# rst-tu-dortmund/mpc_local_planner

Hardware: AMD Instinct MI355X
Metric: MPC solves/sec (batched control cycles) at N=50 carlike (higher is better)
Workload: dtype f64

## Files before the change

mpc_local_planner_amd/csrc/mpc_capi.hip:

```cpp
#include <hip/hip_runtime.h>

#include <cstdio>
#include <cstdlib>
#include <cstring>
#include <new>
#include <string>
#include <vector>

#include "../../include/mpc_hip.h"
#include "mpc_core.hpp"
#include "mpc_problem.hpp"
#include "mpc_launch_plan.hpp"
#include "mpc_wave.hpp"
#include "mpc_solve_kernel.hpp"
#include "mpc_costmap.hpp"
#include "mpc_feasibility.hpp"
#include "mpc_grid_update.hpp"

namespace {

thread_local char g_err[512] = "";

void set_err(const char* what, hipError_t e) {
    snprintf(g_err, sizeof(g_err), "%s: %s", what, hipGetErrorString(e));
// ... 122 lines not shown
    c->model = MPC_MODEL_UNICYCLE;
    c->model_params[0] = 0.5;
    c->model_params[1] = 1.0;
    c->n = 20;
    c->dt_ref = 0.3;
    c->dt_free = 1;
    c->dt_lb = 0.0;
    c->dt_ub = 10.0;
    c->xf_fixed[0] = c->xf_fixed[1] = c->xf_fixed[2] = 1;
    c->collocation = MPC_COLLOC_FORWARD;
    c->objective = MPC_OBJ_MIN_TIME;
    c->u_lb[0] = -0.2; c->u_ub[0] = 0.4;
    c->u_lb[1] = -0.3; c->u_ub[1] = 0.3;
    for (int j = 0; j < 2; ++j) { c->du_lb[j] = -1e30; c->du_ub[j] = 1e30; }
    c->max_iter = 100;
    c->tol = 1e-8;
    c->mu_init = 0.1;
    c->precision = MPC_FP64;
    c->min_obstacle_dist = 0.5;
    c->force_inclusion_dist = 0.5;
    c->cutoff_dist = 2.0;
    c->footprint_kind = MPC_FOOTPRINT_POINT;
    c->max_obstacles = 0;
    c->max_vertices = 1;
    c->max_obstacle_rows = 4;
}

const char* mpc_last_error(void) { return g_err; }
int32_t mpc_version(void) { return 700; }

#ifdef MPC_PROFILE
int mpc_debug_profile(long long* out, int rows) {
#ifdef MPC_SPLIT_BUILD
    std::memset(out, 0, sizeof(long long) * 16 * (size_t)rows);
    hipError_t e = hipSuccess;
#define MPC_PROFILE_ADD(T, M) if (e == hipSuccess) e = mpc::solve_profile_add<T, M>(out, rows);
    MPC_PROFILE_ADD(double, 0) MPC_PROFILE_ADD(double, 1) MPC_PROFILE_ADD(double, 2) MPC_PROFILE_ADD(double, 3)
    MPC_PROFILE_ADD(float, 0) MPC_PROFILE_ADD(float, 1) MPC_PROFILE_ADD(float, 2) MPC_PROFILE_ADD(float, 3)
#undef MPC_PROFILE_ADD
    return (int)e;
#else
    return (int)hipMemcpyFromSymbol(out, HIP_SYMBOL(g_mpc_prof), sizeof(long long) * 16 * (size_t)rows, 0, hipMemcpyDeviceToHost);
#endif
}
#endif

int mpc_create(const mpc_config* cfg, int32_t max_batch, int32_t device, mpc_solver** out) {
    g_err[0] = 0;
    if (!cfg || !out || max_batch <= 0) { set_err("mpc_create: bad argument"); return MPC_EINVAL; }
    *out = nullptr;
    if (const char* why = mpc::config_error(*cfg)) { set_err(why); return MPC_EINVAL; }
    int ndev = 0;
    hipError_t e = hipGetDeviceCount(&ndev);
    if (e != hipSuccess || ndev <= 0) {
        set_err("mpc_create: no HIP device available (this library has no CPU fallback)");
        return MPC_ENODEV;
    }
    if (device < 0 || device >= ndev) { set_err("mpc_create: device index out of range"); return MPC_ENODEV; }
    HIP_TRY(hipSetDevice(device));
    const mpc::LaunchPlan plan = mpc::make_launch_plan(*cfg);
    if (const char* why = mpc::plan_error(plan)) { set_err(why); return MPC_EINVAL; }
    mpc_solver* s = new (std::nothrow) mpc_solver;
    if (!s) return MPC_ENOMEM;
    memset(s, 0, sizeof(*s));
    s->cfg = *cfg;
    s->plan = plan;
    mpc::fill_records(*cfg, s->P64, s->P32);
    s->device = device;
    s->max_batch = max_batch;
    const size_t n = cfg->n;
    hipError_t er = hipStreamCreateWithFlags(&s->stream, hipStreamNonBlocking);
    if (er == hipSuccess) er = hipEventCreate(&s->ev0);
    if (er == hipSuccess) er = hipEventCreate(&s->ev1);
    if (er == hipSuccess) er = hipEventCreate(&s->cev0);
    if (er == hipSuccess) er = hipEventCreate(&s->cev1);
// ... 605 lines not shown
```

mpc_local_planner_amd/csrc/mpc_solve_kernel.hpp:

```cpp
#pragma once
#include <hip/hip_runtime.h>
#include <cstddef>
#include <vector>

#include "../../include/mpc_hip.h"
#include "mpc_core.hpp"
#include "mpc_launch_plan.hpp"
#include "mpc_wave.hpp"

namespace mpc {

struct CandCtl {
    int n_cand;
    int* win;
    int* exited;
    int* it_sum;
    double* rec;
    int32_t* winner_out;
    int32_t* iters_total_out;
    int32_t* rows_dropped;
    double* dual;
    int dual_words;
    int dual_read;
};
// ... 192 lines not shown
    }
    return kern;
}

template <typename T, int MODEL>
hipError_t launch_solve(const SolveLaunch& a) {
    if (a.k.L.GSW > 0 && !a.gstage) return hipErrorInvalidConfiguration;
    auto kern = select_kernel<T, MODEL>(a.k);
    if (!kern) return hipErrorInvalidConfiguration;
    if (a.k.lds > 48u * 1024u) {
        hipError_t e = hipFuncSetAttribute(reinterpret_cast<const void*>(kern), hipFuncAttributeMaxDynamicSharedMemorySize, (int)a.k.lds);
        if (e != hipSuccess) return e;
    }
    hipLaunchKernelGGL(kern, dim3((unsigned)a.B * (unsigned)(a.cc.n_cand > 1 ? a.cc.n_cand : 1)), dim3(kWave), a.k.lds, a.stream, *static_cast<const Problem<T>*>(a.rec), a.k.L, a.B, a.x0, a.xf, a.u_prev, a.dt_prev,
                       a.x_init, a.u_init, a.dt_init, a.obst, a.n_grid, a.n_via, a.via, a.cc, a.iters_add, a.x_out, a.u_out, a.dt_out, a.status, a.iters, a.gstage, a.gslots, a.n_gslots,
                       static_cast<const Problem<T>*>(a.ptab), a.set_of);
    return hipSuccess;
}

template <typename T, int MODEL>
hipError_t solve_occupancy(const KernelChoice& k, int* out) {
    auto kern = select_kernel<T, MODEL>(k);
    if (!kern) return hipErrorInvalidConfiguration;
    if (k.lds > 48u * 1024u) {
        hipError_t e = hipFuncSetAttribute(reinterpret_cast<const void*>(kern), hipFuncAttributeMaxDynamicSharedMemorySize, (int)k.lds);
        if (e != hipSuccess) return e;
    }
    return hipOccupancyMaxActiveBlocksPerMultiprocessor(out, kern, kWave, k.lds);
}

#ifdef MPC_PROFILE
template <typename T, int MODEL>
hipError_t solve_profile_add(long long* acc, int rows) {
    std::vector<long long> b((size_t)16 * rows);
    hipError_t e = hipMemcpyFromSymbol(b.data(), HIP_SYMBOL(g_mpc_prof), sizeof(long long) * b.size(), 0, hipMemcpyDeviceToHost);
    for (size_t i = 0; e == hipSuccess && i < b.size(); ++i) acc[i] += b[i];
    return e;
}
#endif

#if defined(MPC_SPLIT_BUILD) && !defined(MPC_SOLVE_INST)
#ifdef MPC_PROFILE
#define MPC_EXTERN_PROFILE(T, M) extern template hipError_t solve_profile_add<T, M>(long long*, int);
#else
#define MPC_EXTERN_PROFILE(T, M)
#endif
#define MPC_EXTERN_LAUNCH(T, M) extern template hipError_t launch_solve<T, M>(const SolveLaunch&); extern template hipError_t solve_occupancy<T, M>(const KernelChoice&, int*); \
                                MPC_EXTERN_PROFILE(T, M)
MPC_EXTERN_LAUNCH(double, 0) MPC_EXTERN_LAUNCH(double, 1) MPC_EXTERN_LAUNCH(double, 2) MPC_EXTERN_LAUNCH(double, 3)
MPC_EXTERN_LAUNCH(float, 0) MPC_EXTERN_LAUNCH(float, 1) MPC_EXTERN_LAUNCH(float, 2) MPC_EXTERN_LAUNCH(float, 3)
#undef MPC_EXTERN_LAUNCH
#undef MPC_EXTERN_PROFILE
#endif

}
```

mpc_local_planner_amd/csrc/mpc_wave.hpp:

```cpp
#pragma once
#include <hip/hip_runtime.h>
#include <type_traits>

#include "mpc_core.hpp"
#include "mpc_dpp_blocks.inc"

#ifdef MPC_PROFILE
__device__ long long g_mpc_prof[4096][16];
#endif

#include "mpc_wave_layout.hpp"
#include "mpc_wave_debug.hpp"

namespace mpc {

template <typename T, int MODEL, int EXT = 1, bool OBST = true, int NSC = 0, bool GS = false, bool W2 = false>
struct IpmWave {
    static constexpr int NSTG = EXT ? NSTG_EXT : NSTG_BASE;
    static constexpr int NTRB = (MODEL == MODEL_KINEMATIC_BICYCLE || MODEL == MODEL_SIMPLE_CAR_FRONT) ? 4 : 3;
    static_assert(NSC == 0 || (EXT == 0 && !OBST), "the fixed layout exists for the headline instantiation only");
    static_assert(!GS || NSC == 0, "the fixed layout keeps its factorisation data in LDS");
    static_assert(!W2 || (!GS && EXT == 0 && !OBST), "the two-wave kernel exists for the headline instantiation in the LDS form only");
    using LayoutT = typename LayoutOf<NSC, NTRB, NSTG>::type;
    const Problem<T>& P;
    const LayoutT L;
    T* sm;
    T* gmb = nullptr;
    const int lane;
    T x0[3], xf[3], uprev[2], dtprev;
    T mu, rho, delta_last;
    T erho = T(0);
    bool row0_on, fail0;
    bool warm_guess = false;
    mutable int cnt_mult = -1, cnt_bmult = -1;
    mutable T inv_cnt_mult = T(1), inv_cnt_bmult = T(1);
    int nvia = 0;
    int flags;
#ifdef MPC_PROFILE
    mutable long long prof_mult = 0;
    mutable long long prof_loop = 0, prof_setup = 0, prof_fwd_loop = 0;
#endif
// ... 91 lines not shown
    }
    __device__ __forceinline__ T ut(int j, int k, T alpha) const {
        T u = F(L.U, j, k);
        if (alpha != T(0)) u += alpha * F(L.DU, j, k);
        return u;
    }

    __device__ __forceinline__ bool row_on(int r, int q) const { return ron(q) && (r > 0 || row0_on); }

    __device__ __forceinline__ T row_val(int UB, T d, int r, int q) const {
        const int n = L.n, j = q & 1;
        T ur = r < n - 1 ? F(UB, j, r) : T(0);
        const T up0 = uprev[0], up1 = uprev[1];
        T um = j ? up1 : up0;
        if (r > 0) um = F(UB, j, r - 1);
        T dtp = r > 0 ? d : dtprev;
        return slot_sign<T>(q) * ((ur - um) - P.rate_lim[q] * dtp);
    }
    __device__ __forceinline__ T row_jdz(int r, int q, T dd) const {
        const int n = L.n, j = q & 1;
        T dur = r < n - 1 ? F(L.DU, j, r) : T(0);
        T dum = r > 0 ? F(L.DU, j, r - 1) : T(0);
        return slot_sign<T>(q) * ((dur - dum) - (r > 0 ? P.rate_lim[q] * dd : T(0)));
    }

    __device__ __forceinline__ T push_interior(T v, T lb, T ub) const {
        T pl = t_min(Algo<T>::bound_push * t_max(T(1), t_abs(lb)), Algo<T>::bound_push * (ub - lb));
        T pu = t_min(Algo<T>::bound_push * t_max(T(1), t_abs(ub)), Algo<T>::bound_push * (ub - lb));
        return t_min(t_max(v, lb + pl), ub - pu);
    }

    __device__ __forceinline__ int local_lane() const { int l = lane; asm volatile("" : "+v"(l)); return l; }
#define MPC_PHASE_LANE const int lane = W2 ? this->local_lane() : this->lane; (void)lane;
    static constexpr bool kUniformScalars = W2;
    __device__ __forceinline__ static double uni_(double v) { return __hiloint2double(__builtin_amdgcn_readfirstlane(__double2hiint(v)), __builtin_amdgcn_readfirstlane(__double2loint(v))); }
    __device__ __forceinline__ static float uni_(float v) { return __int_as_float(__builtin_amdgcn_readfirstlane(__float_as_int(v))); }
    __device__ __attribute__((noinline)) static T pow_cold(T a, T b) { return t_pow(a, b); }
    __device__ __forceinline__ static T pow_(T a, T b) { if constexpr (W2) return pow_cold(a, b); else return t_pow(a, b); }
    __device__ __forceinline__ static void U(T& v) { if constexpr (kUniformScalars) v = uni_(v); }
    template <typename... Ts> __device__ __forceinline__ static void U(T& v, Ts&... rest) { U(v); U(rest...); }

#include "mpc_wave_rows.inc"
#include "mpc_wave_passes.inc"
#include "mpc_wave_sweeps.inc"
#include "mpc_wave_pit.inc"
#include "mpc_wave_step.inc"
#include "mpc_wave_solve.inc"
#undef MPC_PHASE_LANE
};

}
```

mpc_local_planner_amd/csrc/mpc_wave_debug.hpp:

```cpp
#pragma once

#ifdef MPC_ASM_MARK
#define MPC_MARK(name) asm volatile("; " name)
#else
#define MPC_MARK(name) do { } while (0)
#endif

#ifdef MPC_PROFILE
#define MPC_PROFILE_BEGIN \
        long long tk[8] = {0, 0, 0, 0, 0, 0, 0, 0}; int nfac = 0, ntrial = 0; \
        const long long t_begin = __builtin_readcyclecounter(); \
        const long long w_begin = wall_clock64();
#define MPC_TICK(i, stmt) { long long t0_ = __builtin_readcyclecounter(); stmt; tk[i] += __builtin_readcyclecounter() - t0_; }
#define MPC_PROFILE_COUNT(c) ++c
#define MPC_PROFILE_END \
        if (lane == 0 && blockIdx.x < 4096) { \
            long long* o = g_mpc_prof[blockIdx.x]; \
            o[0] = __builtin_readcyclecounter() - t_begin; o[1] = wall_clock64() - w_begin; o[2] = it; o[3] = nfac; o[4] = ntrial; \
            for (int i = 0; i < 8; ++i) o[5 + i] = tk[i]; \
            o[13] = prof_loop; o[14] = prof_setup; o[15] = prof_fwd_loop; if (prof_mult) o[10] = prof_mult;       \
        }
#else
#define MPC_PROFILE_BEGIN
#define MPC_TICK(i, stmt) { stmt; }
#define MPC_PROFILE_COUNT(c) do { } while (0)
#define MPC_PROFILE_END
#endif

#ifdef MPC_PIT_CHECK
#define MPC_DBG_PIT_CHECK \
                if (pit && (int)blockIdx.x < MPC_PIT_CHECK) { \
                    T dd1 = T(0), nu1[3] = {T(0), T(0), T(0)}, dd2 = T(0), nu2[3] = {T(0), T(0), T(0)}; \
                    const int g1c = backward_pit(delta, dc, dd1, nu1); sync(); \
                    const bool g1 = g1c > 0; \
                    if (g1) { forward_pit(dd1, nu1, delta); sync(); } \
                    T keepx = T(0), keepu = T(0), keepl = T(0); \
                    const int kk = lane < L.n - 1 ? lane : 0; \
                    keepx = F(L.DX, 2, kk); keepu = F(L.DU, 1, kk); keepl = F(L.LAMN, 2, kk); \
                    sync(); \
                    const bool g2 = backward_dpp(delta, dc, dd2, nu2); sync(); \
                    if (g2) { forward_states(dd2, nu2, delta); sync(); } \
                    const T ex = wave_max(t_abs(keepx - F(L.DX, 2, kk))), eu = wave_max(t_abs(keepu - F(L.DU, 1, kk))), el = wave_max(t_abs(keepl - F(L.LAMN, 2, kk))); \
                    const T sx = wave_max(t_abs(F(L.DX, 2, kk))), su = wave_max(t_abs(F(L.DU, 1, kk))), sl = wave_max(t_abs(F(L.LAMN, 2, kk))); \
                    if (lane == 0 && (g1 != g2 || ex > T(1e-7) * (sx + T(1e-3)) || eu > T(1e-7) * (su + T(1e-3)) || el > T(1e-7) * (sl + T(1e-3)))) \
                        printf("blk %d it %d try %d delta %.2e mu %.1e: pit ok %d (code %d) serial ok %d | dd %.9e vs %.9e | max diff dx %.2e (of %.2e) du %.2e (of %.2e) lam %.2e (of %.2e)\n", (int)blockIdx.x, it, ntry, (double)delta, (double)mu, \
                               (int)g1, g1c, (int)g2, (double)dd1, (double)dd2, (double)ex, (double)sx, (double)eu, (double)su, (double)el, (double)sl); \
                    sync(); \
                }
#else
#define MPC_DBG_PIT_CHECK
#endif

#ifdef MPC_NANCHECK
#define MPC_DBG_NANCHECK_FIELDS \
                if (blockIdx.x == MPC_NANCHECK && lane == 0) { \
                    const int offs[] = {L.X, L.U, L.LAM, L.LAMN, L.SR, L.YR, L.PL, L.PU, L.DX, L.DU, L.CC, L.TRIG, L.GAIN, L.STG, L.SC, L.VP, L.ZC, L.total}; \
                    const char* nm[] = {"X", "U", "LAM", "LAMN", "SR", "YR", "PL", "PU", "DX", "DU", "CC", "TRIG", "GAIN", "STG", "SC", "VP", "ZC"}; \
// ... 30 lines not shown
```

mpc_local_planner_amd/csrc/mpc_wave_passes.inc:

```

    __device__ __forceinline__ void eval_point(T d, T& theta_c, T& fobj, T alpha = T(0), bool trial = false) const {
        MPC_PHASE_LANE
        const int n = L.n;
        const T al = trial ? alpha : T(0);
        T th = T(0), fo = T(0);
        if (nM() > 0) {
            for_each_row([&](int k, int m) {
                if (oi(m, k) < 0) return;
                T og = T(0), oax = T(0), oay = T(0);
                if (trial) { og = OB_(0, m, k); oax = OB_(1, m, k); oay = OB_(2, m, k); }
                const T px = xt(0, k, al), py = xt(1, k, al), pth = fpline() ? xt(2, k, al) : T(0);
                T g, a3[3], hk, h3[3];
                obst_row3(k, m, px, py, pth, g, a3, hk, h3, d);
                T s = F(L.OS, m, k);
                if (erho > T(0)) {
                    const T ee = OE_(0, m, k), de = trial ? T(OE_(1, m, k)) : T(0);
                    if (trial) s += alpha * (-(og + s - ee) - obst_jdz(k, m, oax, oay) + de);
                    const T et = ee + (trial ? alpha * de : T(0));
                    th += t_abs(g + s - et);
                    fo += erho * et;
                    return;
                }
                if (trial) s += alpha * (-(og + s) - obst_jdz(k, m, oax, oay));
                th += t_abs(g + s);
// ... 57 lines not shown
            if (nM() > 0 && k >= 1 && k < n - 1) {
                for (int m0 = 0; m0 < nM(); m0 += kRowGroup) {
                RowCache oc;
                if (trial) ob_load<false>(m0, k, oc);
#pragma unroll
                for (int jm = 0; jm < kRowGroup; ++jm) {
                    const int m = m0 + jm;
                    if (m >= nM()) break;
                    if (oi(m, k) < 0) continue;
                    T s = F(L.OS, m, k);
                    if (erho > T(0)) {
                        const T ee = OE_(0, m, k), de = trial ? T(OE_(1, m, k)) : T(0);
                        if (trial) s += alpha * (-(oc.g[jm] + s - ee) - obst_jdz(k, m, oc.ax[jm], oc.ay[jm]) + de);
                        acc.mul(s); acc.mul(ee + (trial ? alpha * de : T(0)));
                        continue;
                    }
                    if (trial) s += alpha * (-(oc.g[jm] + s) - obst_jdz(k, m, oc.ax[jm], oc.ay[jm]));
                    acc.mul(s);
                }
                }
            }
        }
        if (lane == 0 && dtf()) { acc.mul(d - P.dt_lb); acc.mul(P.dt_ub - d); }
        if (lane == 0 && ball()) acc.mul(ball_slack(alpha, trial));
        return wave_sum(acc.value());
    }

    struct TrialRegs {
        T xk[3], dxk[3], xn[3], dxn[3], u[2], du[2], s[4], ds[4];
        T ulb[2], uub[2], dt_lb, dt_ub, nm1;
        bool stage, on[4], quad, mint, dtf;
        int k;
    };
    __device__ __forceinline__ bool trial_fast_ok() const { return EXT == 0 && !GS && !W2 && !OBST && !(sizeof(T) == 8 && NTRB > 3) && L.n <= kWave; }
    __device__ __forceinline__ void trial_setup(TrialRegs& r, T dd) const {
        MPC_PHASE_LANE
        const int n = L.n, k = lane;
        const T d = SCL(SC_D);
        r.k = k; r.stage = k < n - 1;
        r.quad = quad(); r.mint = mintime(); r.dtf = dtf(); r.nm1 = T(n - 1);
        r.dt_lb = P.dt_lb; r.dt_ub = P.dt_ub;
        for (int i = 0; i < 3; ++i) {
            r.xk[i] = r.dxk[i] = r.xn[i] = r.dxn[i] = T(0);
            if (r.stage) {
                r.xk[i] = F(L.X, i, k); r.xn[i] = F(L.X, i, k + 1);
                if (k > 0) r.dxk[i] = F(L.DX, i, k);
                if (k + 1 < n - 1 || !fx(i)) r.dxn[i] = F(L.DX, i, k + 1);
            }
        }
        for (int j = 0; j < 2; ++j) {
            r.ulb[j] = P.u_lb[j]; r.uub[j] = P.u_ub[j];
            r.u[j] = r.stage ? F(L.U, j, k) : T(0); r.du[j] = r.stage ? F(L.DU, j, k) : T(0);
        }
        for (int q = 0; q < 4; ++q) {
            r.on[q] = k < n && row_on(k, q);
            r.s[q] = T(1); r.ds[q] = T(0);
            if (r.on[q]) { const T s = F(L.SR, q, k); r.s[q] = s; r.ds[q] = -(row_val(L.U, d, k, q) + s) - row_jdz(k, q, dd); }
        }
    }
    __device__ __forceinline__ void trial_eval(const TrialRegs& r, T alpha, T d, T& th_out, T& fo_out, T& logs_out) const {
        MPC_PHASE_LANE
        T th = T(0), fo = T(0);
        LogAcc<T> acc;
        if (r.stage) {
            const T x0_ = r.xk[0] + alpha * r.dxk[0], x1_ = r.xk[1] + alpha * r.dxk[1];
            const T x2_ = r.k > 0 ? normalize_theta(r.xk[2] + alpha * r.dxk[2]) : r.xk[2];
            const T n0 = r.xn[0] + alpha * r.dxn[0], n1 = r.xn[1] + alpha * r.dxn[1];
            const T n2 = r.dxn[2] != T(0) ? normalize_theta(r.xn[2] + alpha * r.dxn[2]) : r.xn[2];
            const T v = r.u[0] + alpha * r.du[0], w = r.u[1] + alpha * r.du[1];
            T tr[4], tr2[2], f[3];
            model_trig_colloc<T, MODEL>(P, x2_, v, w, d, tr, tr2);
            colloc_f<T, MODEL>(P, tr, tr2, v, w, f);
            const T c0 = d * f[0] - (n0 - x0_), c1 = d * f[1] - (n1 - x1_), c2 = d * f[2] - normalize_theta(n2 - x2_);
            for (int i = 0; i < NTRB; ++i) F(L.TRIG, i, r.k) = tr[i];
            if (P.collocation == COLLOC_CN) { F(L.TRIG, NTRB, r.k) = tr2[0]; F(L.TRIG, NTRB + 1, r.k) = tr2[1]; }
            C_(0, r.k) = c0; C_(1, r.k) = c1; C_(2, r.k) = c2;
            th = t_abs(c0) + t_abs(c1) + t_abs(c2);
            if (r.quad) {
                const T xd0 = x0_ - xf[0], xd1 = x1_ - xf[1], xd2 = normalize_theta(x2_ - xf[2]);
                fo = (P.Q[0] * xd0 * xd0 + P.Q[1] * xd1 * xd1 + P.Q[2] * xd2 * xd2 + P.R[0] * v * v + P.R[1] * w * w) * (intf() ? d : T(1));
            }
            if (via()) { T vv, vg[3]; via_terms(r.k, x0_, x1_, x2_, vv, vg); fo += vv; }
// ... 347 lines not shown
```

mpc_local_planner_amd/csrc/mpc_wave_solve.inc:

```

    __device__ __forceinline__ T enter_restoration(T& dtheta) {
        const int n = L.n;
        erho = Algo<T>::elastic_rho;
        T esum = T(0), dth = T(0);
        for (int k = lane; k < n - 1; k += kWave) {
            if (k < 1) continue;
            for (int m = 0; m < nM(); ++m) {
                if (oi(m, k) < 0) continue;
                const T g = OB_(0, m, k);
                const T s_old = F(L.OS, m, k);
                const T s = t_max(t_max(-g, Algo<T>::clearance_slack_push), s_old);
                const T ee = t_max(g + s, mu / erho);
                const T y = t_max(t_min(F(L.OY, m, k), T(0.5) * erho), mu / s);
                F(L.OS, m, k) = s; F(L.OY, m, k) = y; OE_(0, m, k) = ee; OE_(1, m, k) = T(0);
                esum += ee;
                dth += t_abs(g + s - ee) - t_abs(g + s_old);
            }
        }
        esum = wave_sum(esum);
        dtheta = wave_sum(dth);
        sync();
        return erho * esum;
    }

    __device__ __forceinline__ SolveStats<T> solve() {
        SolveStats<T> out;
        flags = (P.xf_fixed[0] ? 1 : 0) | (P.xf_fixed[1] ? 2 : 0) | (P.xf_fixed[2] ? 4 : 0) | (P.dt_free ? 8 : 0) | (P.objective == OBJ_QUADRATIC ? 16 : 0) |
                (P.has_Qf ? 32 : 0) | (P.rate_on[0] ? 64 : 0) | (P.rate_on[1] ? 128 : 0) | (P.rate_on[2] ? 256 : 0) | (P.rate_on[3] ? 512 : 0) | (P.ball ? 1024 : 0) | (P.via ? 2048 : 0) | ((P.n_obst > 0 && (P.footprint_kind == 2 || P.footprint_kind == 3 || P.footprint_kind == 4)) ? 4096 : 0) | (P.integral_form ? 8192 : 0) | (P.dyn_obst ? 16384 : 0) | (P.hess_mode ? 32768 : 0) | ((P.objective != OBJ_QUADRATIC || P.hybrid) ? 65536 : 0) | (P.costx ? 131072 : 0);
        flags = __builtin_amdgcn_readfirstlane(flags);
        nfix = (int)fx(0) + (int)fx(1) + (int)fx(2);
        row0_on = dtprev != T(0);
        if (iter_cap <= 0) iter_cap = P.max_iter;
        if (lane < 8) sm[L.ZC + lane] = lane == 4 ? T(1) : T(0);
        if constexpr (GS) {
            if (lane < 8) gw((unsigned)(GlobalStage::ZC + lane)) = lane == 4 ? T(1) : T(0);
            for (int k = lane - GlobalStage::kGuard; k < 4 * GlobalStage::tiles(L.NS) - GlobalStage::kGuard; k += kWave) {
#pragma unroll
                for (int j = 0; j < 6; ++j) TL_(TE_Z + j, k) = j == 3 ? T(1) : T(0);
            }
        }
        if (lane < 12) sm[L.ZI + lane] = lane == 6 ? T(1) : T(0);
        const bool pit = pit_enabled();
        init_point();
        U(mu, rho, delta_last); U(x0[0], x0[1], x0[2]); U(xf[0], xf[1], xf[2]); U(uprev[0], uprev[1], dtprev);
        T theta_c, fobj;
        eval_point(SCL(SC_D), theta_c, fobj);
        U(theta_c, fobj);
        sync();
        int it = 0, status = ST_MAX_ITER, n_acc = 0;
        const long long t_start = P.max_ticks > 0 ? (long long)wall_clock64() : 0ll;
        const T acc_tol = P.acc_tol;
        const int acc_it = P.acc_iter;
        T e0 = T(0), logs_cur = T(0), dc_mu = T(-1), dc_val = T(0);
        T last_alpha = T(0), last_ad = T(0);
        int jam_streak = 0;
        T jam_theta0 = T(0);
        bool endgame = false;
        T mu_max = Algo<T>::mu_max_fact * mu; U(mu_max);
        bool have_logs = false;
        const bool filter = P.line_search == 1;
        T fstate = T(-1);
        int nfilt = 0, fpos = 0;
        static_assert(Algo<T>::flt_cap == 16, "the filter's pairs sit in DPP rows 0 and 1");
        MPC_PROFILE_BEGIN
        while (true) {
            Err er;
            MPC_MARK("KKT_BEGIN");
            MPC_TICK(0, er = kkt_pass());
            U(er.rd, er.rp, er.cmin, er.cmax); U(er.csum, er.sum_mult, er.sum_bmult, er.theta); U(inv_cnt_mult, inv_cnt_bmult);
            MPC_MARK("KKT_END");
            if constexpr (OBST) {
                if (nM() > 0 && erho == T(0) && jam_streak >= Algo<T>::elastic_trigger && er.theta >= Algo<T>::elastic_prog * jam_theta0) {
                    T dth_rows;
                    fobj += enter_restoration(dth_rows);
                    theta_c += dth_rows;
                    rho = T(0); have_logs = false; jam_streak = 0;
                    nfilt = 0; fpos = 0;
                    er = kkt_pass();
                    U(er.rd, er.rp, er.cmin, er.cmax); U(er.csum, er.sum_mult, er.sum_bmult, er.theta); U(theta_c, fobj, erho);
                }
            }
            e0 = err_value(er, T(0)); U(e0);
            if (!t_finite(e0) || !t_finite(er.theta) || !t_finite(er.sum_mult) || !t_finite(er.csum)) { status = ST_NUMERICAL; break; }
            if (e0 <= P.tol) { status = ST_CONVERGED; break; }
            n_acc = (acc_it > 0 && e0 <= acc_tol) ? n_acc + 1 : 0;
            if (acc_it > 0 && n_acc >= acc_it) { status = ST_CONVERGED; break; }
            if (it >= iter_cap) { status = ST_MAX_ITER; break; }
            if (P.max_ticks > 0 && (long long)wall_clock64() - t_start > P.max_ticks) { status = ST_TIME_LIMIT; break; }
            if (win_ptr) {
                const int w = __builtin_amdgcn_readfirstlane(__hip_atomic_load(win_ptr, __ATOMIC_RELAXED, __HIP_MEMORY_SCOPE_AGENT));
                if (w < my_cand) { status = ST_SUPERSEDED; break; }
            }
            if (P.mu_strategy == 1 || endgame) {
                for (int guard = 0; guard < 50; ++guard) {
                    T emu = err_value(er, mu);
                    if (emu <= Algo<T>::kappa_eps * mu && mu > P.tol / T(10)) {
                        mu = t_max(P.tol / T(10), t_min(Algo<T>::kappa_mu * mu, pow_(mu, Algo<T>::theta_mu)));
                        rho = T(0);
                    } else break;
                }
            } else if (it > 0) {
                const T avg = er.csum * inv_cnt_bmult;
                const T a_ = T(1) - t_min(last_alpha, last_ad);
                const T sig = t_min(t_max(a_ * a_ * a_, Algo<T>::sigma_min), T(1));
                T mu_new = t_min(t_max(sig * avg, P.tol / T(10)), mu_max);
                mu_new = t_max(mu_new, t_min(mu, Algo<T>::mu_err_floor * e0));
                if (mu_new <= P.tol) { mu_new = P.tol; endgame = true; }
                if (mu_new != mu) { mu = mu_new; rho = T(0); }
            }
            U(mu, rho);
            MPC_MARK("BARRIER_BEGIN");
            MPC_TICK(1, stage_barrier_terms(); sync());
            MPC_MARK("BARRIER_END");
            T tau = t_max(Algo<T>::tau_min, T(1) - mu);
            if (mu != dc_mu) { dc_mu = mu; dc_val = nfix > 0 ? Algo<T>::delta_c * pow_(mu, Algo<T>::kappa_c) : T(0); }
            U(tau, dc_mu, dc_val);
            const T dc = dc_val;
            T delta = (fail0 && delta_last > T(0)) ? t_max(Algo<T>::delta_min, Algo<T>::kappa_minus * delta_last) : T(0);
            U(delta);
            const bool started_zero = delta == T(0);
            bool ok = false;
            Fwd fw;
            T dd = T(0), nu[3] = {T(0), T(0), T(0)}, curv = T(0);
            for (int ntry = 0; ntry <= 40; ++ntry) {
                bool good, used_pit = false;
                MPC_DBG_PIT_CHECK
                if (pit && mu > pit_floor()) {
                    int gp_;
                    MPC_TICK(2, gp_ = backward_pit(delta, dc, dd, nu); sync());
                    good = used_pit = gp_ > 0;
                    if (gp_ == 0) { MPC_TICK(2, good = backward_dpp(delta, dc, dd, nu); sync()); }
                } else { MPC_TICK(2, good = backward_dpp(delta, dc, dd, nu); sync()); }
                MPC_PROFILE_COUNT(nfac);
                MPC_DBG_NANCHECK_FIELDS
                U(dd, nu[0], nu[1], nu[2]);
                if (good) {
                    if (used_pit) { MPC_TICK(3, forward_pit(dd, nu, delta); sync()); }
                    else { MPC_TICK(3, forward_states(dd, nu, delta); sync()); }
                    MPC_DBG_NANCHECK_STEP
                    MPC_MARK("POST_BEGIN");
                    MPC_TICK(4, fw = post_pass(dd, nu, tau));
                    U(fw.hdz, fw.clam, fw.dz2, fw.dphi); U(fw.a_p, fw.a_d, fw.dzmax, fw.nunu);
                    MPC_MARK("POST_END");
                    good = fw.finite;
                    if (good) {
                        curv = -fw.hdz + fw.clam - dc * fw.nunu; U(curv);
                        ok = true; break;
                    }
                }
                if (delta == T(0)) delta = (delta_last == T(0)) ? Algo<T>::delta_first : t_max(Algo<T>::delta_min, Algo<T>::kappa_minus * delta_last);
                else delta *= (delta_last == T(0)) ? Algo<T>::kappa_plus_first : Algo<T>::kappa_plus;
                U(delta);
                if (delta > Algo<T>::delta_max) break;
            }
            if (!ok) { status = ST_LINSOLVE; break; }
            if constexpr (OBST) {
                if (nM() > 0 && erho == T(0)) {
                    if (fw.a_p < Algo<T>::elastic_ap && er.rp > T(1e-3)) { if (jam_streak == 0) jam_theta0 = er.theta; ++jam_streak; }
                    else jam_streak = 0;
                }
            }
            if (delta > T(0)) delta_last = delta;
            U(delta_last);
            if (started_zero) fail0 = delta > T(0);
            const T theta = er.theta;
            if (!filter && theta > T(0)) {
                T sigma = curv > T(0) ? T(1) : T(0);
                T rho_trial = (fw.dphi + T(0.5) * sigma * curv) / ((T(1) - Algo<T>::rho_frac) * theta);
                if (rho < rho_trial) rho = rho_trial + T(1);
                U(rho);
            }
            T phi0;
            if (!have_logs) { MPC_TICK(5, logs_cur = barrier_logs(SCL(SC_D), T(0), false, dd)); have_logs = true; U(logs_cur); }
            const T rho_ls = filter ? T(0) : rho;
            phi0 = fobj - mu * logs_cur + rho_ls * theta;
            T Dm = fw.dphi - rho_ls * theta;
            T theta_rows = theta - theta_c;
            T alpha = fw.a_p;
            U(phi0, Dm, theta_rows, alpha);
            T a_min = T(0), p_ph = T(0), p_th = T(0), theta_max = T(0), theta_min = T(0);
            if (filter) {
                T theta0 = rd_lane(fstate, 32);
                if (theta0 < T(0)) { theta0 = theta; if (lane == 32) fstate = theta; }
                if (mu != rd_lane(fstate, 33)) { nfilt = 0; fpos = 0; if (lane == 33) fstate = mu; }
                theta_max = Algo<T>::flt_thmax * t_max(T(1), theta0); theta_min = Algo<T>::flt_thmin * t_max(T(1), theta0);
                a_min = Algo<T>::flt_gth;
                if (fw.dphi < T(0)) {
                    a_min = t_min(a_min, Algo<T>::flt_gph * theta / (-fw.dphi));
                    if (theta <= theta_min) {
                        p_ph = pow_cold(-fw.dphi, Algo<T>::flt_sph); p_th = pow_cold(theta, Algo<T>::flt_sth);
                        a_min = t_min(a_min, Algo<T>::flt_delta * p_th / p_ph);
                    }
                }
                a_min = a_min * Algo<T>::flt_gal * fw.a_p;
                theta_max = uni_(theta_max); theta_min = uni_(theta_min); a_min = uni_(a_min); p_ph = uni_(p_ph); p_th = uni_(p_th);
            }
            bool accepted = false, sw_arm = false;
            const bool fast_trials = trial_fast_ok();
            TrialRegs tregs;
            if (fast_trials) { MPC_TICK(5, trial_setup(tregs, dd)); }
            T th_t = T(0), f_t = T(0), lg_t = T(0);
            for (int ls = 0; ls < Algo<T>::max_ls; ++ls) {
                if (ls > 0) { alpha *= T(0.5); U(alpha); }
                const bool below = filter && ls > 0 && alpha < a_min;
                T phit, tht;
                T d_t = SCL(SC_D) + (dtf() ? alpha * SCL(SC_DD) : T(0)); U(d_t);
                MPC_MARK("TRIAL_BEGIN");
                if (fast_trials) {
                    MPC_TICK(6, trial_eval(tregs, alpha, d_t, th_t, f_t, lg_t);
                             tht = th_t + (T(1) - alpha) * theta_rows;
                             phit = f_t - mu * lg_t + rho_ls * tht; sync());
                } else {
                    MPC_TICK(6, eval_point(d_t, th_t, f_t, alpha, true);
                             tht = th_t + (T(1) - alpha) * theta_rows;
                             lg_t = barrier_logs(d_t, alpha, true, dd);
                             phit = f_t - mu * lg_t + rho_ls * tht; sync());
                }
                MPC_MARK("TRIAL_END");
                MPC_PROFILE_COUNT(ntrial);
                U(th_t, f_t, lg_t, phit);
                if (!filter) {
                    if (t_finite(phit) && phit - phi0 - Algo<T>::ls_eps * t_abs(phi0) <= Algo<T>::eta_armijo * alpha * Dm) { accepted = true; break; }
                } else {
                    if (below) break;
                    U(tht);
                    bool okf = t_finite(phit) && tht <= theta_max;
                    if (okf) {
                        const T f_ph = __shfl_xor(fstate, 16);
                        const bool dominated = lane < nfilt && !(tht <= (T(1) - Algo<T>::flt_gth) * fstate || phit <= f_ph - Algo<T>::flt_gph * fstate);
                        okf = __builtin_amdgcn_ballot_w64(dominated) == 0ull;
                    }
                    if (okf) {
                        const bool switching = fw.dphi < T(0) && alpha * p_ph > Algo<T>::flt_delta * p_th;
                        if (theta <= theta_min && switching) {
                            if (phit - phi0 - Algo<T>::ls_eps * t_abs(phi0) <= Algo<T>::flt_eta * alpha * fw.dphi) { accepted = true; sw_arm = true; }
                        } else if (tht <= (T(1) - Algo<T>::flt_gth) * theta || phit <= phi0 - Algo<T>::flt_gph * theta) accepted = true;
                    }
                    if (accepted) break;
                }
            }
            if (filter) {
                if (accepted && !sw_arm) {
                    if (lane == fpos) fstate = theta;
                    if (lane == Algo<T>::flt_cap + fpos) fstate = phi0;
                    fpos = (fpos + 1) & (Algo<T>::flt_cap - 1); nfilt = nfilt < Algo<T>::flt_cap ? nfilt + 1 : Algo<T>::flt_cap;
                }
                if (!accepted) {
                    nfilt = 0; fpos = 0;
                    accepted = t_finite(f_t) && t_finite(lg_t);
                }
            }
            MPC_DBG_NANCHECK_LS_FAILED
            if (acc_tol > T(0) && (!accepted || alpha < T(1e-6) * fw.a_p) && e0 <= acc_tol) { status = ST_CONVERGED; break; }
            if (!accepted && alpha * fw.dzmax < T(1e-14)) { status = ST_LINESEARCH; break; }
            MPC_DBG_NANCHECK_LS
            MPC_MARK("ACCEPT_BEGIN");
            MPC_TICK(7, accept(alpha, fw.a_d); sync());
            MPC_MARK("ACCEPT_END");
            theta_c = th_t; fobj = f_t; logs_cur = lg_t;
            last_alpha = alpha; last_ad = fw.a_d;
            U(theta_c, fobj, logs_cur); U(last_alpha, last_ad);
            ++it;
        }
        MPC_PROFILE_END
        out.status = status; out.iters = it; out.kkt_error = e0; out.objective = fobj;
        return out;
    }
```

mpc_local_planner_amd/csrc/mpc_wave_step.inc:

```

    struct Fwd { T hdz, clam, dz2, dphi, a_p, a_d, dzmax, nunu; bool finite; };

    __device__ __forceinline__ void ftb_ratio(T ival, T dval, T& r) const { r = t_max(r, -dval * ival); }
    __device__ __forceinline__ T ftb_alpha(T r, T tau) const { return r > tau ? tau / r : T(1); }

    __device__ __forceinline__ Fwd post_pass(T dd, const T nu[3], T tau) const {
        MPC_PHASE_LANE
        const int n = L.n;
        const T d = SCL(SC_D);
        T hdz = T(0), clam = T(0), dz2 = T(0), dphi = T(0), r_p = T(0), r_d = T(0), dzmax = T(0);
        if (lane == 0) {
            if (dtf()) {
                T dl = d - P.dt_lb, du = P.dt_ub - d;
                T pl = SCL(SC_PDL), pu = SCL(SC_PDU);
                const T idl = t_rcp(dl), idu = t_rcp(du);
                T gb = -mu * idl + mu * idu;
                hdz += gb * dd; dphi += gb * dd;
                ftb_ratio(idl, dd, r_p); ftb_ratio(idu, -dd, r_p);
                ftb_ratio(t_rcp(pl), mu * idl - pl - (pl * idl) * dd, r_d);
                ftb_ratio(t_rcp(pu), mu * idu - pu + (pu * idu) * dd, r_d);
                dz2 += dd * dd; dzmax = t_max(dzmax, t_abs(dd));
            }
            if (mintime()) { hdz += T(n - 1) * dd; dphi += T(n - 1) * dd; }
            if (ball()) {
                const T jdz = ball_jdz(), s = SCL(SC_TS), y = SCL(SC_TY), res = SCL(SC_TG) + s;
                const T is = t_rcp(s);
                const T sig = y * is, ybar = mu * is + sig * res;
                const T ds = -res - jdz, dy = ybar + sig * jdz - y;
                hdz += ybar * jdz;
                dphi -= (mu * is) * ds;
                ftb_ratio(is, ds, r_p);
                ftb_ratio(t_rcp(y), dy, r_d);
            }
        }
        for (int k = lane; k < n; k += kWave) {
            if (k < n - 1) {
                for (int j = 0; j < 2; ++j) {
                    T u = F(L.U, j, k), du_ = F(L.DU, j, k);
                    T dl = u - P.u_lb[j], du = P.u_ub[j] - u;
                    T pl = F(L.PL, j, k), pu = F(L.PU, j, k);
                    const T idl = t_rcp(dl), idu = t_rcp(du);
                    T gbar = mu * idu - mu * idl + (quad() ? T(2) * P.R[j] * u * (intf() ? d : T(1)) : T(0));
                    if (costx() && quad()) gbar += T(2) * P.Ro * F(L.U, 1 - j, k) * (intf() ? d : T(1));
                    hdz += gbar * du_; dphi += gbar * du_;
                    ftb_ratio(idl, du_, r_p); ftb_ratio(idu, -du_, r_p);
                    ftb_ratio(t_rcp(pl), mu * idl - pl - (pl * idl) * du_, r_d);
                    ftb_ratio(t_rcp(pu), mu * idu - pu + (pu * idu) * du_, r_d);
                    dz2 += du_ * du_; dzmax = t_max(dzmax, t_abs(du_));
                }
                for (int i = 0; i < 3; ++i) {
                    clam += C_(i, k) * F(L.LAMN, i, k);
                }
                if (intf()) {
                    const T xd0 = F(L.X, 0, k) - xf[0], xd1 = F(L.X, 1, k) - xf[1], xd2 = normalize_theta(F(L.X, 2, k) - xf[2]);
                    const T v = F(L.U, 0, k), w = F(L.U, 1, k);
                    T sc = P.Q[0] * xd0 * xd0 + P.Q[1] * xd1 * xd1 + P.Q[2] * xd2 * xd2 + P.R[0] * v * v + P.R[1] * w * w;
                    if (costx()) {
                        const T xd[3] = {xd0, xd1, xd2};
                        sc += offquad(P.Qo, xd) + T(2) * P.Ro * v * w;
                        if (k == 0 && P.trapz) sc -= T(0.5) * fullquad(P.Q, P.Qo, xd);
                    }
                    hdz += sc * dd; dphi += sc * dd;
                }
            }
            if (k >= 1) {
                T vg[3] = {T(0), T(0), T(0)};
                if (via() && k < n - 1) { T vv; via_terms(k, F(L.X, 0, k), F(L.X, 1, k), F(L.X, 2, k), vv, vg); }
                T gxo[3] = {T(0), T(0), T(0)};
                if (costx()) {
                    if (k < n - 1) {
                        if (quad()) {
                            const T xd[3] = {F(L.X, 0, k) - xf[0], F(L.X, 1, k) - xf[1], normalize_theta(F(L.X, 2, k) - xf[2])};
                            offmul(P.Qo, xd, gxo);
                            for (int i = 0; i < 3; ++i) gxo[i] *= T(2) * (intf() ? d : T(1));
                        }
                    } else {
                        T xdT[3], y3[3]; xd_final(T(0), xdT);
                        if (hasqf()) { offmul(P.Qfo, xdT, y3); for (int i = 0; i < 3; ++i) gxo[i] += T(2) * y3[i]; }
                        if (P.trapz) {
                            offmul(P.Qo, xdT, y3);
                            for (int i = 0; i < 3; ++i) gxo[i] += d * (P.Q[i] * xdT[i] + y3[i]);
                            const T sc = T(0.5) * fullquad(P.Q, P.Qo, xdT);
                            hdz += sc * dd; dphi += sc * dd;
                        }
                    }
                }
                for (int i = 0; i < 3; ++i) {
                    if (k < n - 1 || !fx(i)) {
                        T dx = F(L.DX, i, k);
                        dz2 += dx * dx; dzmax = t_max(dzmax, t_abs(dx));
                        T g = vg[i];
                        if (quad() && k < n - 1) { T xd = F(L.X, i, k) - xf[i]; if (i == 2) xd = normalize_theta(xd); g = T(2) * P.Q[i] * xd * (intf() ? d : T(1)); }
                        else if (k == n - 1 && hasqf()) { T xd = F(L.X, i, k) - xf[i]; if (i == 2) xd = normalize_theta(xd); g += T(2) * P.Qf[i] * xd; }
                        g += gxo[i];
                        hdz += g * dx; dphi += g * dx;
                    }
                }
            }
            for (int q = 0; q < 4; ++q) {
                if (!row_on(k, q)) continue;
                T jdz = row_jdz(k, q, dd);
                T s = F(L.SR, q, k), y = F(L.YR, q, k);
                T res = row_val(L.U, d, k, q) + s;
                const T is = t_rcp(s);
                T sig = y * is;
                T ybar = mu * is + sig * res;
                T ds = -res - jdz;
                T dy = ybar + sig * jdz - y;
                hdz += ybar * jdz;
                dphi -= (mu * is) * ds;
                ftb_ratio(is, ds, r_p);
                ftb_ratio(t_rcp(y), dy, r_d);
            }
            if (nM() > 0 && k >= 1 && k < n - 1) {
                for (int m0 = 0; m0 < nM(); m0 += kRowGroup) {
                RowCache oc;
                ob_load<false>(m0, k, oc);
#pragma unroll
                for (int jm = 0; jm < kRowGroup; ++jm) {
                    const int m = m0 + jm;
                    if (m >= nM()) break;
                    if (oi(m, k) < 0) continue;
                    const T jdz = obst_jdz(k, m, oc.ax[jm], oc.ay[jm]);
                    const T s = F(L.OS, m, k), y = F(L.OY, m, k);
                    if (erho > T(0)) {
                        const T ee = OE_(0, m, k);
                        T ds, de, dy, ybar;
                        elastic_steps(s, y, oc.g[jm], ee, jdz, ds, de, dy, ybar);
                        OE_(1, m, k) = de;
                        hdz += ybar * jdz;
                        dphi += -(mu * t_rcp(s)) * ds - (mu * t_rcp(ee)) * de + erho * de;
                        ftb_ratio(t_rcp(s), ds, r_p); ftb_ratio(t_rcp(ee), de, r_p);
                        ftb_ratio(t_rcp(y), dy, r_d); ftb_ratio(t_rcp(erho - y), -dy, r_d);
                        continue;
                    }
                    const T res = oc.g[jm] + s;
                    const T is = t_rcp(s);
                    const T sig = y * is;
                    const T ybar = mu * is + sig * res;
                    const T ds = -res - jdz;
                    const T dy = ybar + sig * jdz - y;
                    hdz += ybar * jdz;
                    dphi -= (mu * is) * ds;
                    ftb_ratio(is, ds, r_p);
                    ftb_ratio(t_rcp(y), dy, r_d);
// ... 315 lines not shown
```

Before: 296,700.

## Fuse trial-register setup into post pass and hoist uniform solver scalars

For the headline instantiation, the post pass now records the per-lane control, slack and step values that the line-search trial evaluation needs. This removes the separate trial_setup pass and its reloads from LDS. The loop-invariant problem parameters (tol, max_ticks, mu strategy, line search) are hoisted into readfirstlane-uniform locals, and uniform-scalar broadcasting is enabled for the non-extended, obstacle-free kernel. Profiling gains gap counters and more columns. The risks are higher register pressure in post_pass and a register lifetime for tregs that now spans the factorisation retries.

```diff
diff --git a/mpc_local_planner_amd/csrc/mpc_capi.hip b/mpc_local_planner_amd/csrc/mpc_capi.hip
--- a/mpc_local_planner_amd/csrc/mpc_capi.hip
+++ b/mpc_local_planner_amd/csrc/mpc_capi.hip
@@ -178,7 +178,7 @@
 #ifdef MPC_PROFILE
 int mpc_debug_profile(long long* out, int rows) {
 #ifdef MPC_SPLIT_BUILD
-    std::memset(out, 0, sizeof(long long) * 16 * (size_t)rows);
+    std::memset(out, 0, sizeof(long long) * mpc::kProfCols * (size_t)rows);
     hipError_t e = hipSuccess;
 #define MPC_PROFILE_ADD(T, M) if (e == hipSuccess) e = mpc::solve_profile_add<T, M>(out, rows);
     MPC_PROFILE_ADD(double, 0) MPC_PROFILE_ADD(double, 1) MPC_PROFILE_ADD(double, 2) MPC_PROFILE_ADD(double, 3)
@@ -186,7 +186,7 @@
 #undef MPC_PROFILE_ADD
     return (int)e;
 #else
-    return (int)hipMemcpyFromSymbol(out, HIP_SYMBOL(g_mpc_prof), sizeof(long long) * 16 * (size_t)rows, 0, hipMemcpyDeviceToHost);
+    return (int)hipMemcpyFromSymbol(out, HIP_SYMBOL(g_mpc_prof), sizeof(long long) * mpc::kProfCols * (size_t)rows, 0, hipMemcpyDeviceToHost);
 #endif
 }
 #endif
diff --git a/mpc_local_planner_amd/csrc/mpc_solve_kernel.hpp b/mpc_local_planner_amd/csrc/mpc_solve_kernel.hpp
--- a/mpc_local_planner_amd/csrc/mpc_solve_kernel.hpp
+++ b/mpc_local_planner_amd/csrc/mpc_solve_kernel.hpp
@@ -248,7 +248,7 @@
 #ifdef MPC_PROFILE
 template <typename T, int MODEL>
 hipError_t solve_profile_add(long long* acc, int rows) {
-    std::vector<long long> b((size_t)16 * rows);
+    std::vector<long long> b((size_t)kProfCols * rows);
     hipError_t e = hipMemcpyFromSymbol(b.data(), HIP_SYMBOL(g_mpc_prof), sizeof(long long) * b.size(), 0, hipMemcpyDeviceToHost);
     for (size_t i = 0; e == hipSuccess && i < b.size(); ++i) acc[i] += b[i];
     return e;
diff --git a/mpc_local_planner_amd/csrc/mpc_wave.hpp b/mpc_local_planner_amd/csrc/mpc_wave.hpp
--- a/mpc_local_planner_amd/csrc/mpc_wave.hpp
+++ b/mpc_local_planner_amd/csrc/mpc_wave.hpp
@@ -6,7 +6,8 @@
 #include "mpc_dpp_blocks.inc"
 
 #ifdef MPC_PROFILE
-__device__ long long g_mpc_prof[4096][16];
+namespace mpc { constexpr int kProfCols = 24, kProfTicks = 14; }
+__device__ long long g_mpc_prof[4096][mpc::kProfCols];
 #endif
 
 #include "mpc_wave_layout.hpp"
@@ -164,9 +165,11 @@
 
     __device__ __forceinline__ int local_lane() const { int l = lane; asm volatile("" : "+v"(l)); return l; }
 #define MPC_PHASE_LANE const int lane = W2 ? this->local_lane() : this->lane; (void)lane;
-    static constexpr bool kUniformScalars = W2;
+    static constexpr bool kUniformScalars = W2 || (EXT == 0 && !OBST && !GS);
     __device__ __forceinline__ static double uni_(double v) { return __hiloint2double(__builtin_amdgcn_readfirstlane(__double2hiint(v)), __builtin_amdgcn_readfirstlane(__double2loint(v))); }
     __device__ __forceinline__ static float uni_(float v) { return __int_as_float(__builtin_amdgcn_readfirstlane(__float_as_int(v))); }
+    __device__ __forceinline__ static int uni_(int v) { return __builtin_amdgcn_readfirstlane(v); }
+    __device__ __forceinline__ static long long uni_(long long v) { return ((long long)__builtin_amdgcn_readfirstlane((int)(v >> 32)) << 32) | (unsigned)__builtin_amdgcn_readfirstlane((int)v); }
     __device__ __attribute__((noinline)) static T pow_cold(T a, T b) { return t_pow(a, b); }
     __device__ __forceinline__ static T pow_(T a, T b) { if constexpr (W2) return pow_cold(a, b); else return t_pow(a, b); }
     __device__ __forceinline__ static void U(T& v) { if constexpr (kUniformScalars) v = uni_(v); }
diff --git a/mpc_local_planner_amd/csrc/mpc_wave_debug.hpp b/mpc_local_planner_amd/csrc/mpc_wave_debug.hpp
--- a/mpc_local_planner_amd/csrc/mpc_wave_debug.hpp
+++ b/mpc_local_planner_amd/csrc/mpc_wave_debug.hpp
@@ -8,21 +8,24 @@
 
 #ifdef MPC_PROFILE
 #define MPC_PROFILE_BEGIN \
-        long long tk[8] = {0, 0, 0, 0, 0, 0, 0, 0}; int nfac = 0, ntrial = 0; \
+        long long tk[mpc::kProfTicks] = {}; int nfac = 0, ntrial = 0; \
         const long long t_begin = __builtin_readcyclecounter(); \
+        long long t_lap = t_begin; \
         const long long w_begin = wall_clock64();
-#define MPC_TICK(i, stmt) { long long t0_ = __builtin_readcyclecounter(); stmt; tk[i] += __builtin_readcyclecounter() - t0_; }
+#define MPC_TICK(i, stmt) { long long t0_ = __builtin_readcyclecounter(); stmt; t_lap = __builtin_readcyclecounter(); tk[i] += t_lap - t0_; }
+#define MPC_GAP_END(i) { const long long t1_ = __builtin_readcyclecounter(); tk[i] += t1_ - t_lap; t_lap = t1_; }
 #define MPC_PROFILE_COUNT(c) ++c
 #define MPC_PROFILE_END \
         if (lane == 0 && blockIdx.x < 4096) { \
             long long* o = g_mpc_prof[blockIdx.x]; \
             o[0] = __builtin_readcyclecounter() - t_begin; o[1] = wall_clock64() - w_begin; o[2] = it; o[3] = nfac; o[4] = ntrial; \
-            for (int i = 0; i < 8; ++i) o[5 + i] = tk[i]; \
-            o[13] = prof_loop; o[14] = prof_setup; o[15] = prof_fwd_loop; if (prof_mult) o[10] = prof_mult;       \
+            for (int i = 0; i < mpc::kProfTicks; ++i) o[5 + i] = tk[i]; \
+            o[19] = prof_loop; o[20] = prof_setup; o[21] = prof_fwd_loop; if (prof_mult) o[10] = prof_mult;       \
         }
 #else
 #define MPC_PROFILE_BEGIN
 #define MPC_TICK(i, stmt) { stmt; }
+#define MPC_GAP_END(i) do { } while (0)
 #define MPC_PROFILE_COUNT(c) do { } while (0)
 #define MPC_PROFILE_END
 #endif
diff --git a/mpc_local_planner_amd/csrc/mpc_wave_passes.inc b/mpc_local_planner_amd/csrc/mpc_wave_passes.inc
--- a/mpc_local_planner_amd/csrc/mpc_wave_passes.inc
+++ b/mpc_local_planner_amd/csrc/mpc_wave_passes.inc
@@ -113,11 +113,10 @@
         bool stage, on[4], quad, mint, dtf;
         int k;
     };
-    __device__ __forceinline__ bool trial_fast_ok() const { return EXT == 0 && !GS && !W2 && !OBST && !(sizeof(T) == 8 && NTRB > 3) && L.n <= kWave; }
-    __device__ __forceinline__ void trial_setup(TrialRegs& r, T dd) const {
-        MPC_PHASE_LANE
-        const int n = L.n, k = lane;
-        const T d = SCL(SC_D);
+    static constexpr bool kFusedPasses = EXT == 0 && !GS && !W2 && !OBST && !(sizeof(T) == 8 && NTRB > 3);
+    __device__ __forceinline__ bool trial_fast_ok() const { if constexpr (NSC > 0 && NSC <= kWave) return kFusedPasses; else return kFusedPasses && L.n <= kWave; }
+    __device__ __forceinline__ void trial_setup_states(TrialRegs& r, int k) const {
+        const int n = L.n;
         r.k = k; r.stage = k < n - 1;
         r.quad = quad(); r.mint = mintime(); r.dtf = dtf(); r.nm1 = T(n - 1);
         r.dt_lb = P.dt_lb; r.dt_ub = P.dt_ub;
@@ -129,6 +128,12 @@
                 if (k + 1 < n - 1 || !fx(i)) r.dxn[i] = F(L.DX, i, k + 1);
             }
         }
+    }
+    __device__ __forceinline__ void trial_setup(TrialRegs& r, T dd) const {
+        MPC_PHASE_LANE
+        const int n = L.n, k = lane;
+        const T d = SCL(SC_D);
+        trial_setup_states(r, k);
         for (int j = 0; j < 2; ++j) {
             r.ulb[j] = P.u_lb[j]; r.uub[j] = P.u_ub[j];
             r.u[j] = r.stage ? F(L.U, j, k) : T(0); r.du[j] = r.stage ? F(L.DU, j, k) : T(0);
diff --git a/mpc_local_planner_amd/csrc/mpc_wave_solve.inc b/mpc_local_planner_amd/csrc/mpc_wave_solve.inc
--- a/mpc_local_planner_amd/csrc/mpc_wave_solve.inc
+++ b/mpc_local_planner_amd/csrc/mpc_wave_solve.inc
@@ -48,9 +48,12 @@
         U(theta_c, fobj);
         sync();
         int it = 0, status = ST_MAX_ITER, n_acc = 0;
-        const long long t_start = P.max_ticks > 0 ? (long long)wall_clock64() : 0ll;
-        const T acc_tol = P.acc_tol;
-        const int acc_it = P.acc_iter;
+        const T tol = uni_(P.tol), tol10 = uni_(P.tol / T(10));
+        const bool mu_monotone = uni_(P.mu_strategy) == 1;
+        const long long max_ticks = uni_(P.max_ticks);
+        const long long t_start = max_ticks > 0 ? (long long)wall_clock64() : 0ll;
+        const T acc_tol = uni_(P.acc_tol);
+        const int acc_it = uni_(P.acc_iter);
         T e0 = T(0), logs_cur = T(0), dc_mu = T(-1), dc_val = T(0);
         T last_alpha = T(0), last_ad = T(0);
         int jam_streak = 0;
@@ -58,13 +61,14 @@
         bool endgame = false;
         T mu_max = Algo<T>::mu_max_fact * mu; U(mu_max);
         bool have_logs = false;
-        const bool filter = P.line_search == 1;
+        const bool filter = uni_(P.line_search) == 1;
         T fstate = T(-1);
         int nfilt = 0, fpos = 0;
         static_assert(Algo<T>::flt_cap == 16, "the filter's pairs sit in DPP rows 0 and 1");
         MPC_PROFILE_BEGIN
         while (true) {
             Err er;
+            MPC_GAP_END(13);
             MPC_MARK("KKT_BEGIN");
             MPC_TICK(0, er = kkt_pass());
             U(er.rd, er.rp, er.cmin, er.cmax); U(er.csum, er.sum_mult, er.sum_bmult, er.theta); U(inv_cnt_mult, inv_cnt_bmult);
@@ -82,20 +86,20 @@
             }
             e0 = err_value(er, T(0)); U(e0);
             if (!t_finite(e0) || !t_finite(er.theta) || !t_finite(er.sum_mult) || !t_finite(er.csum)) { status = ST_NUMERICAL; break; }
-            if (e0 <= P.tol) { status = ST_CONVERGED; break; }
+            if (e0 <= tol) { status = ST_CONVERGED; break; }
             n_acc = (acc_it > 0 && e0 <= acc_tol) ? n_acc + 1 : 0;
             if (acc_it > 0 && n_acc >= acc_it) { status = ST_CONVERGED; break; }
             if (it >= iter_cap) { status = ST_MAX_ITER; break; }
-            if (P.max_ticks > 0 && (long long)wall_clock64() - t_start > P.max_ticks) { status = ST_TIME_LIMIT; break; }
+            if (max_ticks > 0 && (long long)wall_clock64() - t_start > max_ticks) { status = ST_TIME_LIMIT; break; }
             if (win_ptr) {
                 const int w = __builtin_amdgcn_readfirstlane(__hip_atomic_load(win_ptr, __ATOMIC_RELAXED, __HIP_MEMORY_SCOPE_AGENT));
                 if (w < my_cand) { status = ST_SUPERSEDED; break; }
             }
-            if (P.mu_strategy == 1 || endgame) {
+            if (mu_monotone || endgame) {
                 for (int guard = 0; guard < 50; ++guard) {
                     T emu = err_value(er, mu);
-                    if (emu <= Algo<T>::kappa_eps * mu && mu > P.tol / T(10)) {
-                        mu = t_max(P.tol / T(10), t_min(Algo<T>::kappa_mu * mu, pow_(mu, Algo<T>::theta_mu)));
+                    if (emu <= Algo<T>::kappa_eps * mu && mu > tol10) {
+                        mu = t_max(tol10, t_min(Algo<T>::kappa_mu * mu, pow_(mu, Algo<T>::theta_mu)));
                         rho = T(0);
                     } else break;
                 }
@@ -103,12 +107,13 @@
                 const T avg = er.csum * inv_cnt_bmult;
                 const T a_ = T(1) - t_min(last_alpha, last_ad);
                 const T sig = t_min(t_max(a_ * a_ * a_, Algo<T>::sigma_min), T(1));
-                T mu_new = t_min(t_max(sig * avg, P.tol / T(10)), mu_max);
+                T mu_new = t_min(t_max(sig * avg, tol10), mu_max);
                 mu_new = t_max(mu_new, t_min(mu, Algo<T>::mu_err_floor * e0));
-                if (mu_new <= P.tol) { mu_new = P.tol; endgame = true; }
+                if (mu_new <= tol) { mu_new = tol; endgame = true; }
                 if (mu_new != mu) { mu = mu_new; rho = T(0); }
             }
             U(mu, rho);
+            MPC_GAP_END(9);
             MPC_MARK("BARRIER_BEGIN");
             MPC_TICK(1, stage_barrier_terms(); sync());
             MPC_MARK("BARRIER_END");
@@ -121,25 +126,29 @@
             const bool started_zero = delta == T(0);
             bool ok = false;
             Fwd fw;
+            TrialRegs tregs;
             T dd = T(0), nu[3] = {T(0), T(0), T(0)}, curv = T(0);
             for (int ntry = 0; ntry <= 40; ++ntry) {
                 bool good, used_pit = false;
                 MPC_DBG_PIT_CHECK
+                MPC_GAP_END(10);
                 if (pit && mu > pit_floor()) {
                     int gp_;
                     MPC_TICK(2, gp_ = backward_pit(delta, dc, dd, nu); sync());
                     good = used_pit = gp_ > 0;
-                    if (gp_ == 0) { MPC_TICK(2, good = backward_dpp(delta, dc, dd, nu); sync()); }
+                    if (gp_ == 0) { MPC_GAP_END(10); MPC_TICK(2, good = backward_dpp(delta, dc, dd, nu); sync()); }
                 } else { MPC_TICK(2, good = backward_dpp(delta, dc, dd, nu); sync()); }
                 MPC_PROFILE_COUNT(nfac);
                 MPC_DBG_NANCHECK_FIELDS
                 U(dd, nu[0], nu[1], nu[2]);
                 if (good) {
+                    MPC_GAP_END(10);
                     if (used_pit) { MPC_TICK(3, forward_pit(dd, nu, delta); sync()); }
                     else { MPC_TICK(3, forward_states(dd, nu, delta); sync()); }
                     MPC_DBG_NANCHECK_STEP
+                    MPC_GAP_END(10);
                     MPC_MARK("POST_BEGIN");
-                    MPC_TICK(4, fw = post_pass(dd, nu, tau));
+                    MPC_TICK(4, fw = post_pass<kFusedPasses>(dd, nu, tau, tregs));
                     U(fw.hdz, fw.clam, fw.dz2, fw.dphi); U(fw.a_p, fw.a_d, fw.dzmax, fw.nunu);
                     MPC_MARK("POST_END");
                     good = fw.finite;
@@ -171,7 +180,7 @@
                 U(rho);
             }
             T phi0;
-            if (!have_logs) { MPC_TICK(5, logs_cur = barrier_logs(SCL(SC_D), T(0), false, dd)); have_logs = true; U(logs_cur); }
+            if (!have_logs) { MPC_GAP_END(11); MPC_TICK(5, logs_cur = barrier_logs(SCL(SC_D), T(0), false, dd)); have_logs = true; U(logs_cur); }
             const T rho_ls = filter ? T(0) : rho;
             phi0 = fobj - mu * logs_cur + rho_ls * theta;
             T Dm = fw.dphi - rho_ls * theta;
@@ -197,14 +206,17 @@
             }
             bool accepted = false, sw_arm = false;
             const bool fast_trials = trial_fast_ok();
-            TrialRegs tregs;
-            if (fast_trials) { MPC_TICK(5, trial_setup(tregs, dd)); }
+            MPC_GAP_END(11);
+            MPC_MARK("TSETUP_BEGIN");
+            if (fast_trials && !kFusedPasses) { MPC_TICK(8, trial_setup(tregs, dd)); }
+            MPC_MARK("TSETUP_END");
             T th_t = T(0), f_t = T(0), lg_t = T(0);
             for (int ls = 0; ls < Algo<T>::max_ls; ++ls) {
                 if (ls > 0) { alpha *= T(0.5); U(alpha); }
                 const bool below = filter && ls > 0 && alpha < a_min;
                 T phit, tht;
                 T d_t = SCL(SC_D) + (dtf() ? alpha * SCL(SC_DD) : T(0)); U(d_t);
+                MPC_GAP_END(11);
                 MPC_MARK("TRIAL_BEGIN");
                 if (fast_trials) {
                     MPC_TICK(6, trial_eval(tregs, alpha, d_t, th_t, f_t, lg_t);
@@ -254,6 +266,7 @@
             if (acc_tol > T(0) && (!accepted || alpha < T(1e-6) * fw.a_p) && e0 <= acc_tol) { status = ST_CONVERGED; break; }
             if (!accepted && alpha * fw.dzmax < T(1e-14)) { status = ST_LINESEARCH; break; }
             MPC_DBG_NANCHECK_LS
+            MPC_GAP_END(12);
             MPC_MARK("ACCEPT_BEGIN");
             MPC_TICK(7, accept(alpha, fw.a_d); sync());
             MPC_MARK("ACCEPT_END");
diff --git a/mpc_local_planner_amd/csrc/mpc_wave_step.inc b/mpc_local_planner_amd/csrc/mpc_wave_step.inc
--- a/mpc_local_planner_amd/csrc/mpc_wave_step.inc
+++ b/mpc_local_planner_amd/csrc/mpc_wave_step.inc
@@ -4,11 +4,17 @@
     __device__ __forceinline__ void ftb_ratio(T ival, T dval, T& r) const { r = t_max(r, -dval * ival); }
     __device__ __forceinline__ T ftb_alpha(T r, T tau) const { return r > tau ? tau / r : T(1); }
 
-    __device__ __forceinline__ Fwd post_pass(T dd, const T nu[3], T tau) const {
+    template <bool REC>
+    __device__ __forceinline__ Fwd post_pass(T dd, const T nu[3], T tau, TrialRegs& tr) const {
         MPC_PHASE_LANE
         const int n = L.n;
         const T d = SCL(SC_D);
         T hdz = T(0), clam = T(0), dz2 = T(0), dphi = T(0), r_p = T(0), r_d = T(0), dzmax = T(0);
+        if constexpr (REC) {
+            trial_setup_states(tr, lane);
+            for (int j = 0; j < 2; ++j) { tr.ulb[j] = P.u_lb[j]; tr.uub[j] = P.u_ub[j]; tr.u[j] = tr.du[j] = T(0); }
+            for (int q = 0; q < 4; ++q) { tr.on[q] = false; tr.s[q] = T(1); tr.ds[q] = T(0); }
+        }
         if (lane == 0) {
             if (dtf()) {
                 T dl = d - P.dt_lb, du = P.dt_ub - d;
@@ -47,6 +53,7 @@
                     ftb_ratio(t_rcp(pl), mu * idl - pl - (pl * idl) * du_, r_d);
                     ftb_ratio(t_rcp(pu), mu * idu - pu + (pu * idu) * du_, r_d);
                     dz2 += du_ * du_; dzmax = t_max(dzmax, t_abs(du_));
+                    if constexpr (REC) { tr.u[j] = u; tr.du[j] = du_; }
                 }
                 for (int i = 0; i < 3; ++i) {
                     clam += C_(i, k) * F(L.LAMN, i, k);
@@ -111,6 +118,7 @@
                 dphi -= (mu * is) * ds;
                 ftb_ratio(is, ds, r_p);
                 ftb_ratio(t_rcp(y), dy, r_d);
+                if constexpr (REC) { tr.on[q] = true; tr.s[q] = s; tr.ds[q] = ds; }
             }
             if (nM() > 0 && k >= 1 && k < n - 1) {
                 for (int m0 = 0; m0 < nM(); m0 += kRowGroup) {
```

New measurement: 307,800, median of 6. 3.7% higher.
